# AlanLiangC/PDM-SSD

Measured on AMD Instinct MI355X. Metric: frames/sec (16384-pt clouds, bs=32), higher is better.
Workload: dtype f32; 1 GPU; configs[2]: full PDM-SSD forward (PointNet2MSG backbone + PDM neck + hybrid head: BEV heat-map head + point box head with decoded boxes), bs=32/GPU x 16384 pts, uniform KITTI-range clouds, fp32 inference, inputs resident in HBM, 4 distinct batches in rotation; launch=hipGraph, parallelism=dp1, global_batch=32

## Files before the change

### include/pdmssd_hip.h

```cpp
#ifndef PDMSSD_HIP_H
#define PDMSSD_HIP_H

#include <stddef.h>

#ifdef __cplusplus
extern "C" {
#endif

#define PDM_ABI_VERSION 1

#define PDM_E_BADARG (-1)
#define PDM_E_TOOLARGE (-2)

int pdm_abi_version(void);
const char *pdm_last_error(void);


int pdm_ball_query(void *stream, int b, int n, int m, float radius, int nsample,
                   const float *new_xyz, const float *xyz, int *idx);

int pdm_group_points(void *stream, int b, int c, int n, int npoints, int nsample,
                     const float *points, const int *idx, float *out);

int pdm_group_points_grad(void *stream, int b, int c, int n, int npoints, int nsample,
// ... 330 lines not shown
                        void *xmin, unsigned char *imax, unsigned char *imin);
int pdm_tg_dy_stats_parts(long long rows, int N);
int pdm_tg_gemm_nt_dy_bs(void *stream, long long R, int K, int N, const void *dZ, long long lddz, const void *Yp, long long ldyp,
                         const void *W, long long ldw, void *dX, long long lddx, void *dYout, long long lddy, const float *coef,
                         const float *grads, const void *Bx, long long ldbx, const float *bcoef, float *bstats);
size_t pdm_tg_wgrad_ws_bytes(long long R, int K, int N);
int pdm_tg_wgrad(void *stream, long long R, int K, int N, const void *dY, long long ldy, const void *X, long long ldx, float *dW,
                 int accumulate, void *workspace, size_t workspace_bytes, const float *x_bn_coef);
size_t pdm_tg_colsum_ws_floats(long long R, int N);
int pdm_tg_colsum(void *stream, long long R, int N, const void *Y, long long ld, float *out, float *scratch);
int pdm_tg_pack_weight(void *stream, int N, int K, const float *W, void *Wb, int ldb, void *Wt, int ldt);
int pdm_tg_pack_weight_pair(void *stream, int N, int K, const float *W, void *Wb, void *Wt, int rows_to, int cols_to);
int pdm_tg_pack_weight_many(void *stream, int njobs, const void *jobs, long long total_blocks);


int pdm_tune_fps_variant(int v);
int pdm_tune_fused_waves(int w);
int pdm_tune_fused_tiles(int t);
int pdm_tune_fused_groups(int n);
int pdm_tune_fused_wg_per_cu(int n);
int pdm_tune_fused_lds_cap(int bytes);
int pdm_tune_fused_reg(int on);
int pdm_tune_fused_gemm(int on);
int pdm_tune_fused_chain(int on);
int pdm_tune_fused_swz(int on);
int pdm_tune_bq_quad(int form);
int pdm_tune_bq_dense_ppc(int hundredths);
int pdm_tune_grid_split(int min_n);
int pdm_tune_bq_small_waves(int w);
int pdm_tune_bq_cpw(int centres);
int pdm_tune_bq_heavy(int candidates);
int pdm_tune_group_lds_floor(int bytes);
int pdm_tune_group_rows(int packed);
int pdm_tune_rows_chain_wg_per_cu(int n);
int pdm_tune_fp_head_tiles(int n);
int pdm_tune_rows_chain_dw_wg_per_cu(int n);
int pdm_tune_rows_chain_xcd(int on);
int pdm_tune_fp_chain_pad_lds(int bytes);

int pdm_copy_many(void *stream, int count, void *const *dst, const void *const *src, const size_t *bytes);
int pdm_copy_many_dyn(void *stream, int count, void *const *dst, const void *const *src, const size_t *bytes,
                      const int *const *dyn_count, const unsigned *dyn_unit);


int pdm_scatter_bev(void *stream, int B, int P, int C, int degree, const float *xyz,
                    const float *feat, const float *sh, const float *inv2s2, float ox, float oy,
// ... 37 lines not shown
```

### pdm_ssd_amd/_native.py

```python
import ctypes
import os

import torch

_HERE = os.path.dirname(os.path.abspath(__file__))
LIB_PATH = os.path.join(_HERE, "libpdmssd_hip.so")
ABI_VERSION = 1

_lib = None

_vp, _i, _f = ctypes.c_void_p, ctypes.c_int, ctypes.c_float

_SIGNATURES = {
    "pdm_ball_query": [_i, _i, _i, _f, _i, _vp, _vp, _vp],
    "pdm_ball_query_grid": [_i, _i, _i, _f, _i, _vp, _vp, _vp, _vp, ctypes.c_size_t],
    "pdm_grid_build": [_i, _i, _f, _vp, _vp, ctypes.c_size_t],
    "pdm_ball_query_grid_prebuilt": [_i, _i, _i, _f, _i, _vp, _vp, _vp, ctypes.c_size_t],
    "pdm_three_nn_grid_prebuilt": [_i, _i, _i, _vp, _vp, _vp, _vp, ctypes.c_size_t],
    "pdm_three_nn_grid": [_i, _i, _i, _vp, _vp, _vp, _vp, _vp, ctypes.c_size_t],
    "pdm_group_points": [_i, _i, _i, _i, _i, _vp, _vp, _vp],
    "pdm_group_points_grad": [_i, _i, _i, _i, _i, _vp, _vp, _vp],
    "pdm_group_points_grad_ws": [_i, _i, _i, _i, _i, _vp, _vp, _vp, _vp, ctypes.c_size_t],
    "pdm_gather_points": [_i, _i, _i, _i, _vp, _vp, _vp],
    "pdm_gather_points_grad": [_i, _i, _i, _i, _vp, _vp, _vp],
# ... 111 lines not shown
    "pdm_tg_colsum": [ctypes.c_longlong, _i, _vp, ctypes.c_longlong, _vp, _vp],
    "pdm_tg_pack_weight": [_i, _i, _vp, _vp, _i, _vp, _i],
    "pdm_tg_pack_weight_pair": [_i, _i, _vp, _vp, _vp, _i, _i],
    "pdm_tg_pack_weight_many": [_i, _vp, ctypes.c_longlong],
    "pdm_tune_fps_variant": None,
    "pdm_tune_fused_waves": None,
    "pdm_tune_fused_tiles": None,
    "pdm_tune_fused_groups": None,
    "pdm_tune_fused_wg_per_cu": None,
    "pdm_tune_fused_lds_cap": None,
    "pdm_tune_fused_reg": None,
    "pdm_tune_bq_quad": None,
    "pdm_tune_bq_heavy": None,
    "pdm_tune_bq_cpw": None,
    "pdm_tune_copy_variant": None,
    "pdm_tune_group_nt": None,
    "pdm_tune_group_lds_floor": None,
    "pdm_tune_copy_max_wg": None,
    "pdm_tune_bq_small_waves": None,
    "pdm_tune_bq_dense_ppc": None,
    "pdm_tune_grid_split": None,
    "pdm_tune_group_rows": None,
    "pdm_tune_fused_gemm": None,
    "pdm_tune_fused_chain": None,
    "pdm_tune_fused_pair": None,
    "pdm_tune_sa_pair": None,
    "pdm_tune_rows_x3_wg_per_cu": None,
    "pdm_tune_fp_chain_pad_lds": None,
    "pdm_tune_fp_chain_nt": None,
    "pdm_tune_fp_chain_mask": None,
    "pdm_tune_rows_chain_wg_per_cu": None,
    "pdm_tune_rows_chain_dw_wg_per_cu": None,
    "pdm_tune_fp_head_tiles": None,
    "pdm_tune_rows_chain_xcd": None,
    "pdm_tune_fused_swz": None,
    "pdm_scatter_bev": [_i, _i, _i, _i, _vp, _vp, _vp, _vp] + [_f] * 9 + [_i] * 7 + [_vp, _vp],
    "pdm_gather_bev": [_i, _i, _i, _i, _vp, _vp, _vp, _vp] + [_f] * 9 + [_i] * 6 + [_i, _f, _vp, _vp, _vp, ctypes.c_size_t],
    "pdm_bev_normalize_grad": [_i, _i, _i, _i, _i, _f, _vp, _vp, _vp, _vp, _vp],
    "pdm_bev_normalize": [_i, _i, _i, _i, _i, _i, _f, _vp, _vp],
    "pdm_scatter_bev_grad": [_i, _i, _i, _i, _vp, _vp, _vp, _vp] + [_f] * 9 + [_i] * 7 + [_vp] * 5,
    "pdm_scatter_bev_grad_normalized": [_i, _i, _i, _i, _vp, _vp, _vp, _vp] + [_f] * 9 + [_i] * 7 + [_vp, _vp, _f] + [_vp] * 4,
}
EXPORTS = ["pdm_abi_version", "pdm_last_error", "pdm_ball_query_grid_workspace_bytes",
           "pdm_three_nn_grid_workspace_bytes", "pdm_furthest_point_sampling_ws_bytes",
           "pdm_fps_max_coresident_workgroups",
           "pdm_gather_bev_workspace_bytes", "pdm_nms_workspace_bytes", "pdm_post_process_workspace_bytes", "pdm_augment_workspace_bytes", "pdm_kitti_eval_workspace_bytes", "pdm_kitti_data_fov_workspace_bytes",
           "pdm_kitti_data_boxes_workspace_bytes", "pdm_sa_pack_workspace_bytes",
           "pdm_sa_pack_rows", "pdm_rows_mlp_x3_stream_bytes", "pdm_point_head_loss_workspace_bytes", "pdm_heatmap_focal_loss_workspace_bytes", "pdm_three_interpolate_grad_ws_bytes",
           "pdm_group_points_grad_ws_bytes", "pdm_group_concat_cl_grad_ws_bytes", "pdm_bn_parts", "pdm_bn_pool_parts",
           "pdm_tg_stats_parts", "pdm_tg_dy_stats_parts", "pdm_tg_wgrad_ws_bytes", "pdm_tg_colsum_ws_floats"] + list(_SIGNATURES)


class NativeLibraryError(RuntimeError):
    pass


def lib():
    global _lib
    if _lib is None:
        if not os.path.exists(LIB_PATH):
            raise NativeLibraryError(
                f"{LIB_PATH} not found: build it with `make -C pdm_ssd_amd/csrc` "
                "(or `python -c 'import __graft_entry__ as g; g.build()'`). "
                "pdm_ssd_amd has no CPU or PyTorch fallback for its operators.")
        l = ctypes.CDLL(LIB_PATH)
        l.pdm_abi_version.restype = _i
        l.pdm_last_error.restype = ctypes.c_char_p
        l.pdm_ball_query_grid_workspace_bytes.restype = ctypes.c_size_t
        l.pdm_ball_query_grid_workspace_bytes.argtypes = [_i, _i]
        l.pdm_furthest_point_sampling_ws_bytes.restype = ctypes.c_size_t
        l.pdm_furthest_point_sampling_ws_bytes.argtypes = [_i, _i]
        l.pdm_fps_max_coresident_workgroups.restype = _i
        l.pdm_fps_max_coresident_workgroups.argtypes = []
        l.pdm_gather_bev_workspace_bytes.restype = ctypes.c_size_t
        l.pdm_gather_bev_workspace_bytes.argtypes = [_i] * 6
        l.pdm_three_nn_grid_workspace_bytes.restype = ctypes.c_size_t
        l.pdm_three_nn_grid_workspace_bytes.argtypes = [_i, _i]
        l.pdm_nms_workspace_bytes.restype = ctypes.c_size_t
        l.pdm_sa_pack_workspace_bytes.restype = ctypes.c_size_t
        l.pdm_sa_pack_workspace_bytes.argtypes = [_i, _i]
        l.pdm_group_concat_cl_grad_ws_bytes.restype = ctypes.c_size_t
        l.pdm_group_concat_cl_grad_ws_bytes.argtypes = [_i, _i, _i, _i]
        l.pdm_group_points_grad_ws_bytes.restype = ctypes.c_size_t
        l.pdm_group_points_grad_ws_bytes.argtypes = [_i, _i, _i, _i]
        l.pdm_three_interpolate_grad_ws_bytes.restype = ctypes.c_size_t
        l.pdm_three_interpolate_grad_ws_bytes.argtypes = [_i, _i, _i]
        l.pdm_point_head_loss_workspace_bytes.restype = ctypes.c_size_t
        l.pdm_point_head_loss_workspace_bytes.argtypes = [ctypes.c_longlong]
        l.pdm_heatmap_focal_loss_workspace_bytes.restype = ctypes.c_size_t
        l.pdm_heatmap_focal_loss_workspace_bytes.argtypes = [ctypes.c_longlong]
        l.pdm_rows_mlp_x3_stream_bytes.restype = ctypes.c_size_t
        l.pdm_rows_mlp_x3_stream_bytes.argtypes = [_i, _vp]
        l.pdm_sa_pack_rows.restype = ctypes.c_size_t
        l.pdm_sa_pack_rows.argtypes = [_i, _i, _i]
        l.pdm_nms_workspace_bytes.argtypes = [_i]
        l.pdm_post_process_workspace_bytes.restype = ctypes.c_size_t
# ... 102 lines not shown
```

### pdm_ssd_amd/csrc/fused_mlp.hip

```cpp
#include "common.h"

#include <mutex>
#include <set>

namespace pdm {

typedef float f4 __attribute__((ext_vector_type(4)));

constexpr int FM_MAXL = 4;

struct MlpDesc {
    int nlayers;
    int K[FM_MAXL + 1];
    int woff[FM_MAXL];
    int boff[FM_MAXL];
    int stage_in;
    int pool_floats;
    int relu_last;
    int lds_p, lds_q;
    int swz;
};

__device__ __forceinline__ int lds_col(int blk, int g, int pos, int swz) {
    const int q = 4 * blk + g;
// ... 976 lines not shown
            for (int t = 0; t < NT; ++t)
                if (orow[t]) sa_reg_store4(orow[t], 16 * mb + 4 * g, a.cout, v[t]);
        }
    }
}

int rows_gemm_launch(void *stream, int rows, int cin, const float *in_pm, int k0, int c1, const float *wpack,
                     const float *bias, int relu_last, float *out_pm, int out_stride, int cout);
int rows_chain_launch(void *stream, int rows, int cin, const float *in_pm, int nlayers, const int *dims, const float *wpack,
                      const float *bias, int relu_last, float *out_pm, int out_stride, int cout, int *launched);
int rows_chain_pair_launch(void *stream, int rows, int cin, const float *in_pm, int nlayers, const int *dims, const float *wpack_a,
                           const float *bias_a, const float *wpack_b, const float *bias_b, int relu_last, float *out_a, int out_stride_a,
                           int cout_a, float *out_b, int out_stride_b, int cout_b, int *launched);
static int g_fused_chain = 1;
static int g_fused_pair = 1;
int fp_chain_launch(void *stream, int b, int n, int m, int c_skip, const float *z_pm, int z_stride, const float *skip_pm,
                    const int *idx, const float *weight, const int *dims, const float *wpack, const float *bias, float *out_pm,
                    int out_stride, int cout, int *launched);
int fp_pre_gemm_launch(void *stream, int b, int n, int m, int c_skip, const float *z_pm, int z_stride,
                       const float *skip_pm, const int *idx, const float *weight, int k1, int c2,
                       const float *wpack, const float *bias, float *out_pm, int out_stride, int cout);
static int g_fused_swz = 1;
static int g_fused_gemm = 1;
static int g_fused_reg = 1;
static int g_fused_waves = 0;
static int g_fused_tiles = 0;
static int g_fused_groups = 0;
static int g_fused_lds_cap = 152 * 1024;
static int g_fused_wg_per_cu = 32;

static int fill_desc(const char *who, MlpDesc &d, int nlayers, const int *dims, int k0_real_max, int pool_floats,
                     long long ntiles, int *waves, int *tiles_per_wg, int *groups, bool two_tiles) {
    PDM_REQUIRE(nlayers >= 1 && nlayers <= FM_MAXL, PDM_E_BADARG, "%s: nlayers=%d not in [1,%d]", who, nlayers, FM_MAXL);
    PDM_REQUIRE(dims, PDM_E_BADARG, "%s: null dims", who);
    d.nlayers = nlayers;
    d.relu_last = 1;
    int wo = 0, bo = 0;
    for (int l = 0; l <= nlayers; ++l) {
        PDM_REQUIRE(dims[l] > 0 && dims[l] % 16 == 0, PDM_E_BADARG, "%s: padded width %d of level %d is not a positive multiple of 16", who, dims[l], l);
        d.K[l] = dims[l];
    }
    for (int l = 0; l < nlayers; ++l) {
        d.woff[l] = wo; d.boff[l] = bo;
        wo += d.K[l] * d.K[l + 1];
        bo += d.K[l + 1];
    }
// ... 20 lines not shown
    d.lds_q = roww(q);
    d.pool_floats = pool_floats;
    const int region_bytes = (NT * 16 * (d.lds_p + d.lds_q) + pool_floats) * 4;
    int G = NT == 2 ? 1 : (g_fused_groups > 0 ? g_fused_groups : W == 2 ? 2 : 1);
    while (G > 1 && (G * W > 8 || (long long)G * region_bytes > 64 * 1024 || (long long)G * NT * 4 > ntiles)) G >>= 1;
    *groups = G;
    return 0;
}

}

using namespace pdm;

extern "C" int pdm_tune_fused_waves(int w) { const int old = g_fused_waves; g_fused_waves = (w == 1 || w == 2 || w == 4 || w == 8) ? w : 0; return old; }

static void allow_lds(const void *fn, size_t bytes) {
    if (bytes > 64 * 1024) (void)grant_lds(fn, 160 * 1024);
}
extern "C" int pdm_tune_fused_lds_cap(int bytes) { const int old = g_fused_lds_cap; if (bytes >= 16 * 1024 && bytes <= 160 * 1024) g_fused_lds_cap = bytes; return old; }
extern "C" int pdm_tune_fused_swz(int on) { const int old = g_fused_swz; g_fused_swz = on != 0; return old; }
extern "C" int pdm_tune_fused_chain(int on) { const int old = g_fused_chain; g_fused_chain = on != 0; return old; }
extern "C" int pdm_tune_fused_pair(int on) { const int old = g_fused_pair; g_fused_pair = on != 0; return old; }
extern "C" int pdm_tune_fused_gemm(int on) { const int old = g_fused_gemm; g_fused_gemm = on != 0; return old; }
extern "C" int pdm_tune_fused_reg(int on) { const int old = g_fused_reg; g_fused_reg = on != 0; return old; }
extern "C" int pdm_tune_fused_wg_per_cu(int n) { const int old = g_fused_wg_per_cu; if (n > 0) g_fused_wg_per_cu = n; return old; }
extern "C" int pdm_tune_fused_groups(int n) { const int old = g_fused_groups; g_fused_groups = (n == 1 || n == 2 || n == 4 || n == 8) ? n : 0; return old; }
extern "C" int pdm_tune_fused_tiles(int t) { const int old = g_fused_tiles; g_fused_tiles = t; return old; }

#define FUSED_LAUNCH2(KERNEL, W, G, PRE, blocks, lds_bytes, ...)                                              \
    do {                                                                                                       \
        constexpr int MAXNB = (W <= 2) ? 2 : 4;      \
        if (NT == 2 && W >= 4 && G == 1) {                           \
            allow_lds(reinterpret_cast<const void *>(&KERNEL<(W >= 4 ? W : 4), 2, 2, 1, PRE>), lds_bytes);     \
            hipLaunchKernelGGL((KERNEL<(W >= 4 ? W : 4), 2, 2, 1, PRE>), dim3(blocks), dim3(64 * W * G),       \
                               lds_bytes, as_stream(stream), __VA_ARGS__);                                     \
        } else {                                                                                               \
            allow_lds(reinterpret_cast<const void *>(&KERNEL<W, 1, MAXNB, G, PRE>), lds_bytes);                \
            hipLaunchKernelGGL((KERNEL<W, 1, MAXNB, G, PRE>), dim3(blocks), dim3(64 * W * G), lds_bytes,       \
                               as_stream(stream), __VA_ARGS__);                                                \
        }                                                                                                      \
    } while (0)
#define FUSED_LAUNCH1(KERNEL, W, G, blocks, lds_bytes, ...)                                                   \
    do {                                                                                                       \
        if (pre_form) FUSED_LAUNCH2(KERNEL, W, G, true, blocks, lds_bytes, __VA_ARGS__);                       \
        else FUSED_LAUNCH2(KERNEL, W, G, false, blocks, lds_bytes, __VA_ARGS__);                               \
    } while (0)
// ... 199 lines not shown
    int rc = fill_desc("fp_mlp_fused", d, nlayers, dims, c_known + c_skip, 0, ntiles, &W, &NT, &G, mode == 1);
    if (rc) return rc;
    d.relu_last = relu_last ? 1 : 0;
    if (mode == 1)
        PDM_REQUIRE(z_stride % 4 == 0 && z_stride >= d.K[1] && (reinterpret_cast<uintptr_t>(z_pm) & 15) == 0, PDM_E_BADARG,
                    "fp_mlp_fused_pre: z rows need %d floats, stride %d, 16-byte aligned", d.K[1], z_stride);
    PDM_REQUIRE(cout > 0 && cout <= d.K[nlayers] && cout <= out_stride, PDM_E_BADARG, "fp_mlp_fused: cout=%d stride=%d", cout, out_stride);
    PDM_REQUIRE(out_stride % 4 == 0 && (reinterpret_cast<uintptr_t>(out_pm) & 15) == 0 &&
                    (reinterpret_cast<uintptr_t>(wpack) & 15) == 0 && (reinterpret_cast<uintptr_t>(bias) & 15) == 0 &&
                    (c_known % 4 != 0 || (reinterpret_cast<uintptr_t>(known_pm) & 15) == 0) &&
                    (c_skip % 4 != 0 || c_skip == 0 || (reinterpret_cast<uintptr_t>(skip_pm) & 15) == 0),
                PDM_E_BADARG, "fp_mlp_fused: buffers must be 16-byte aligned and out_stride a multiple of 4");
    FpArgs a{b, n, m, c_known, c_skip, known_pm, skip_pm, idx, weight, out_pm, out_stride, cout, mode == 1 ? z_pm : nullptr, z_stride};
    const bool pre_form = mode == 1;
    PDM_REQUIRE(!pre_form || (long long)m * z_stride < (1ll << 31), PDM_E_TOOLARGE, "fp_mlp_fused_pre: m * z_stride overflows 32-bit row offsets");
    if (g_fused_chain && pre_form && nlayers == 2 && z_stride >= d.K[1] &&
        (c_skip <= 4 || (c_skip % 4 == 0 && (reinterpret_cast<uintptr_t>(skip_pm) & 15) == 0))) {
        int launched = 0;
        const int crc = fp_chain_launch(stream, b, n, m, c_skip, z_pm, z_stride, skip_pm, idx, weight, dims, wpack, bias, out_pm,
                                        out_stride, cout, &launched);
        if (crc || launched) return crc;
    }
    if (g_fused_gemm && pre_form && nlayers == 2 && c_skip <= 4 && d.K[0] == 16 && d.K[1] >= 64 && d.K[2] >= 64 &&
        (long long)b * n >= 32768 && (long long)b * n < (1ll << 31) && z_stride >= d.K[1])
        return fp_pre_gemm_launch(stream, b, n, m, c_skip, z_pm, z_stride, skip_pm, idx, weight, d.K[1], d.K[2], wpack, bias,
                                  out_pm, out_stride, cout);
    const size_t lds_bytes = (size_t)G * (NT * 16 * (d.lds_p + d.lds_q)) * sizeof(float);
    PDM_REQUIRE(lds_bytes <= 160 * 1024, PDM_E_TOOLARGE, "fp_mlp_fused: needs %zu bytes of LDS", lds_bytes);
    const long long niter = ((ntiles + NT - 1) / NT + G - 1) / G;
    const long long cap = (long long)256 * g_fused_wg_per_cu;
    const int blocks = (int)(niter < cap ? niter : cap);
    FUSED_DISPATCH(fp_mlp_fused_kernel, W, G, blocks, lds_bytes, d, a, wpack, bias);
    return check_launch("fp_mlp_fused");
}

extern "C" int pdm_fp_mlp_fused(void *stream, int b, int n, int m, int c_known, int c_skip,
                                const float *known_pm, const float *skip_pm, const int *idx,
                                const float *weight, int nlayers, const int *dims, const float *wpack,
                                const float *bias, float *out_pm, int out_stride, int cout) {
    PDM_REQUIRE(c_known >= 1, PDM_E_BADARG, "fp_mlp_fused: c_known=%d", c_known);
    return fp_fused_launch(stream, 0, 1, b, n, m, c_known, c_skip, known_pm, nullptr, 0, skip_pm, idx, weight, nlayers,
                           dims, wpack, bias, out_pm, out_stride, cout);
}

extern "C" int pdm_fp_mlp_fused_pre(void *stream, int b, int n, int m, int c_skip, const float *z_pm,
                                    int z_stride, const float *skip_pm, const int *idx, const float *weight,
                                    int nlayers, const int *dims, const float *wpack, const float *bias,
                                    float *out_pm, int out_stride, int cout) {
    return fp_fused_launch(stream, 1, 1, b, n, m, 0, c_skip, nullptr, z_pm, z_stride, skip_pm, idx, weight, nlayers, dims,
                           wpack, bias, out_pm, out_stride, cout);
}

extern "C" int pdm_rows_mlp_fused(void *stream, int rows, int cin, const float *in_pm, int nlayers,
                                  const int *dims, const float *wpack, const float *bias, int relu_last,
                                  float *out_pm, int out_stride, int cout) {
    PDM_REQUIRE(rows >= 0 && cin >= 1, PDM_E_BADARG, "rows_mlp_fused: rows=%d cin=%d", rows, cin);
    if (g_fused_chain && dims && in_pm && wpack && bias && out_pm && cout > 0 && nlayers >= 1 && nlayers <= 3 && cout <= dims[nlayers] &&
        cout <= out_stride && out_stride % 4 == 0 &&
        ((reinterpret_cast<uintptr_t>(out_pm) | reinterpret_cast<uintptr_t>(wpack) | reinterpret_cast<uintptr_t>(bias) |
          reinterpret_cast<uintptr_t>(in_pm)) & 15) == 0) {
        int launched = 0;
        const int rc = rows_chain_launch(stream, rows, cin, in_pm, nlayers, dims, wpack, bias, relu_last, out_pm, out_stride, cout,
                                         &launched);
        if (rc || launched) return rc;
    }
    if (g_fused_gemm && nlayers == 1 && dims && dims[0] % 16 == 0 && dims[1] % 16 == 0 && dims[0] >= cin && dims[0] >= 32 &&
        dims[1] >= 64 && (long long)((rows + 127) / 128) * ((dims[1] + 127) / 128) >= 256 && in_pm && wpack && bias && out_pm && cout > 0 && cout <= dims[1] && cout <= out_stride &&
        out_stride % 4 == 0 && ((reinterpret_cast<uintptr_t>(out_pm) | reinterpret_cast<uintptr_t>(wpack) |
                                 reinterpret_cast<uintptr_t>(bias)) & 15) == 0)
        return rows_gemm_launch(stream, rows, cin, in_pm, dims[0], dims[1], wpack, bias, relu_last, out_pm, out_stride, cout);
    return fp_fused_launch(stream, 2, relu_last, 1, rows, 1, 0, cin, nullptr, nullptr, 0, in_pm, nullptr, nullptr, nlayers,
                           dims, wpack, bias, out_pm, out_stride, cout);
}

extern "C" int pdm_rows_mlp_fused_pair(void *stream, int rows, int cin, const float *in_pm, int nlayers, const int *dims,
                                       const float *wpack_a, const float *bias_a, const float *wpack_b, const float *bias_b,
                                       int relu_last, float *out_a, int out_stride_a, int cout_a, float *out_b, int out_stride_b,
                                       int cout_b) {
    PDM_REQUIRE(rows >= 0 && cin >= 1, PDM_E_BADARG, "rows_mlp_fused_pair: rows=%d cin=%d", rows, cin);
    if (g_fused_chain && g_fused_pair && dims && in_pm && wpack_a && bias_a && wpack_b && bias_b && out_a && out_b && out_a != out_b &&
        nlayers == 3 && cout_a > 0 && cout_b > 0 && cout_a <= dims[nlayers] && cout_b <= dims[nlayers] && cout_a <= out_stride_a &&
        cout_b <= out_stride_b && out_stride_a % 4 == 0 && out_stride_b % 4 == 0 &&
        ((reinterpret_cast<uintptr_t>(out_a) | reinterpret_cast<uintptr_t>(out_b) | reinterpret_cast<uintptr_t>(wpack_a) |
          reinterpret_cast<uintptr_t>(wpack_b) | reinterpret_cast<uintptr_t>(bias_a) | reinterpret_cast<uintptr_t>(bias_b) |
          reinterpret_cast<uintptr_t>(in_pm)) & 15) == 0) {
        int launched = 0;
        const int rc = rows_chain_pair_launch(stream, rows, cin, in_pm, nlayers, dims, wpack_a, bias_a, wpack_b, bias_b, relu_last, out_a,
                                              out_stride_a, cout_a, out_b, out_stride_b, cout_b, &launched);
        if (rc || launched) return rc;
    }
// ... 4 lines not shown
```

### pdm_ssd_amd/csrc/rows_gemm.hip

```cpp
#include "common.h"

namespace pdm {

typedef float gf4 __attribute__((ext_vector_type(4)));

constexpr int RG_ROWS = 128;
constexpr int RG_BLKS = 8;
constexpr int RG_HS = 24;

struct RowsGemmArgs {
    int rows, cin, in_stride;
    int nkb, nmb;
    int cout, out_stride;
    const float *in;
    const float *wpack;
    const float *bias;
    float *out;
    float floor;
    int n, m, z_stride, c_skip;
    const float *z;
    const float *skip;
    const int *idx;
    const float *weight;
    const float *w1;
    const float *b1;
};

template <bool FP_PRE>
__global__ __launch_bounds__(512) void rows_gemm_kernel(RowsGemmArgs a) {
    __shared__ __attribute__((aligned(16))) float s_w[2][RG_BLKS * 64 * 4];
    __shared__ __attribute__((aligned(16))) float s_h[2][RG_ROWS * RG_HS];
    const int tid = threadIdx.x, lane = tid & 63;
    const int wave = __builtin_amdgcn_readfirstlane(tid >> 6);
    const int pos = lane & 15, g = lane >> 4;
    const int wp = wave >> 2, wc = wave & 3;
    int tile = blockIdx.x;
    if constexpr (FP_PRE) {
        const int tpc = a.n / RG_ROWS, nb = a.rows / a.n;
        if (gridDim.y == 1 && tpc * RG_ROWS == a.n && (nb & 7) == 0) {
            const int xcd = tile & 7, slot = tile >> 3;
            tile = ((slot / tpc) * 8 + xcd) * tpc + slot % tpc;
        }
    }
    const long long r0 = (long long)tile * RG_ROWS;
    const int mb0 = blockIdx.y * RG_BLKS;

    const int hrow = tid >> 2, part = tid & 3;
    const bool w_live = mb0 + wave < a.nmb;
    const gf4 *wsrc = reinterpret_cast<const gf4 *>(a.wpack) + ((size_t)(mb0 + wave) * a.nkb) * 64 + lane;
    const bool h_live = r0 + hrow < a.rows;
    const float *hsrc = a.in + (size_t)(r0 + hrow) * a.in_stride + 4 * part;
    const bool vec = (a.in_stride & 3) == 0 && (reinterpret_cast<uintptr_t>(a.in) & 15) == 0;

    auto load_w = [&](int kb) {
        gf4 v = {0.f, 0.f, 0.f, 0.f};
        if (w_live) v = wsrc[(size_t)kb * 64];
        return v;
    };
    const float *zb = nullptr;
    int o0 = 0, o1 = 0, o2 = 0;
    float iw0 = 0.f, iw1 = 0.f, iw2 = 0.f, sk[4] = {0.f, 0.f, 0.f, 0.f};
    if constexpr (FP_PRE) {
        if (h_live) {
            const long long row = r0 + hrow;
            const int b = (int)(row / a.n);
            zb = a.z + (size_t)b * a.m * a.z_stride + 4 * part;
            o0 = a.idx[row * 3] * a.z_stride; o1 = a.idx[row * 3 + 1] * a.z_stride; o2 = a.idx[row * 3 + 2] * a.z_stride;
            iw0 = a.weight[row * 3]; iw1 = a.weight[row * 3 + 1]; iw2 = a.weight[row * 3 + 2];
            for (int s_ = 0; s_ < a.c_skip; ++s_) sk[s_] = a.skip[row * a.c_skip + s_];
        }
    }
    struct Raw { gf4 za, zc, zd; };
    auto load_raw = [&](int kb) {
        Raw r;
        r.za = r.zc = r.zd = gf4{0.f, 0.f, 0.f, 0.f};
        if (h_live) {
            r.za = *reinterpret_cast<const gf4 *>(zb + o0 + 16 * kb);
            r.zc = *reinterpret_cast<const gf4 *>(zb + o1 + 16 * kb);
            r.zd = *reinterpret_cast<const gf4 *>(zb + o2 + 16 * kb);
        }
        return r;
    };
    auto finish = [&](const Raw &r, int kb) {
        gf4 v = {0.f, 0.f, 0.f, 0.f};
        if (!h_live) return v;
        const int c = 16 * kb + 4 * part;
        const gf4 bb = *reinterpret_cast<const gf4 *>(a.b1 + c);
        float h[4] = {bb.x, bb.y, bb.z, bb.w};
        const float zz[3][4] = {{r.za.x, r.za.y, r.za.z, r.za.w}, {r.zc.x, r.zc.y, r.zc.z, r.zc.w}, {r.zd.x, r.zd.y, r.zd.z, r.zd.w}};
#pragma unroll
        for (int j = 0; j < 4; ++j) {
            h[j] += __fmaf_rn(iw2, zz[2][j], __fmaf_rn(iw1, zz[1][j], __fmul_rn(iw0, zz[0][j])));
            const float *wr = a.w1 + ((size_t)(c >> 4) * 64 + ((c & 15) + j)) * 4;
            for (int s_ = 0; s_ < a.c_skip; ++s_) h[j] = fmaf(wr[s_], sk[s_], h[j]);
            h[j] = fmaxf(h[j], 0.0f);
        }
        return gf4{h[0], h[1], h[2], h[3]};
    };
    auto load_h = [&](int kb) {
        gf4 v = {0.f, 0.f, 0.f, 0.f};
        if (!h_live) return v;
        const int c = 16 * kb + 4 * part;
        if (vec && c + 4 <= a.cin) return *reinterpret_cast<const gf4 *>(hsrc + 16 * kb);
        const float *p = hsrc + 16 * kb;
        if (c < a.cin) v.x = p[0];
        if (c + 1 < a.cin) v.y = p[1];
        if (c + 2 < a.cin) v.z = p[2];
        if (c + 3 < a.cin) v.w = p[3];
        return v;
    };
    auto stage = [&](int buf, gf4 w, gf4 h) {
        reinterpret_cast<gf4 *>(s_w[buf])[tid] = w;
        *reinterpret_cast<gf4 *>(&s_h[buf][hrow * RG_HS + 4 * part]) = h;
    };

    gf4 acc[2][4];
#pragma unroll
    for (int i = 0; i < 2; ++i) {
        gf4 bi = {0.f, 0.f, 0.f, 0.f};
        if (mb0 + 2 * wc + i < a.nmb) bi = *reinterpret_cast<const gf4 *>(a.bias + 16 * (mb0 + 2 * wc + i) + 4 * g);
#pragma unroll
        for (int t = 0; t < 4; ++t) acc[i][t] = bi;
    }

    gf4 gw = load_w(0), gh = {0.f, 0.f, 0.f, 0.f};
    Raw gr;
    if constexpr (FP_PRE) { gr = load_raw(0); gh = finish(gr, 0); } else gh = load_h(0);
    stage(0, gw, gh);
    __syncthreads();
    if (a.nkb > 1) {
        gw = load_w(1);
        if constexpr (FP_PRE) gr = load_raw(1); else gh = load_h(1);
    }
    for (int kb = 0; kb < a.nkb; ++kb) {
        const int cur = kb & 1;
        gf4 fa[2], fb[4];
#pragma unroll
        for (int i = 0; i < 2; ++i) fa[i] = reinterpret_cast<const gf4 *>(s_w[cur])[(2 * wc + i) * 64 + lane];
#pragma unroll
        for (int t = 0; t < 4; ++t) fb[t] = *reinterpret_cast<const gf4 *>(&s_h[cur][((4 * wp + t) * 16 + pos) * RG_HS + 4 * g]);
        if (kb + 1 < a.nkb) {
            if constexpr (FP_PRE) gh = finish(gr, kb + 1);
            stage(cur ^ 1, gw, gh);
        }
        if (kb + 2 < a.nkb) {
            gw = load_w(kb + 2);
            if constexpr (FP_PRE) gr = load_raw(kb + 2); else gh = load_h(kb + 2);
        }
#define PDM_RG_MFMA(C)                                                                                         \
    _Pragma("unroll") for (int i = 0; i < 2; ++i) _Pragma("unroll") for (int t = 0; t < 4; ++t)                 \
        acc[i][t] = __builtin_amdgcn_mfma_f32_16x16x4f32(fa[i].C, fb[t].C, acc[i][t], 0, 0, 0);
        PDM_RG_MFMA(x) PDM_RG_MFMA(y) PDM_RG_MFMA(z) PDM_RG_MFMA(w)
#undef PDM_RG_MFMA
        __syncthreads();
    }

#pragma unroll
    for (int t = 0; t < 4; ++t) {
        const long long row = r0 + (4 * wp + t) * 16 + pos;
        if (row >= a.rows) continue;
        float *orow = a.out + (size_t)row * a.out_stride;
#pragma unroll
        for (int i = 0; i < 2; ++i) {
            const int c0 = 16 * (mb0 + 2 * wc + i) + 4 * g;
            gf4 v = acc[i][t];
            v.x = __builtin_amdgcn_fmed3f(v.x, a.floor, __builtin_inff()); v.y = __builtin_amdgcn_fmed3f(v.y, a.floor, __builtin_inff());
            v.z = __builtin_amdgcn_fmed3f(v.z, a.floor, __builtin_inff()); v.w = __builtin_amdgcn_fmed3f(v.w, a.floor, __builtin_inff());
            if (c0 + 4 <= a.cout) {
                *reinterpret_cast<gf4 *>(orow + c0) = v;
            } else {
                if (c0 < a.cout) orow[c0] = v.x;
                if (c0 + 1 < a.cout) orow[c0 + 1] = v.y;
                if (c0 + 2 < a.cout) orow[c0 + 2] = v.z;
            }
        }
    }
}

int rows_gemm_launch(void *stream, int rows, int cin, const float *in_pm, int k0, int c1, const float *wpack,
                     const float *bias, int relu_last, float *out_pm, int out_stride, int cout) {
    RowsGemmArgs a;
    a.rows = rows; a.cin = cin; a.in_stride = cin;
    a.nkb = k0 >> 4; a.nmb = c1 >> 4;
    a.cout = cout; a.out_stride = out_stride;
    a.in = in_pm; a.wpack = wpack; a.bias = bias; a.out = out_pm;
    a.floor = relu_last ? 0.0f : -__builtin_inff();
    a.n = a.m = a.z_stride = a.c_skip = 0;
    a.z = a.skip = a.weight = a.w1 = a.b1 = nullptr; a.idx = nullptr;
    const dim3 grid((unsigned)((rows + RG_ROWS - 1) / RG_ROWS), (unsigned)((a.nmb + RG_BLKS - 1) / RG_BLKS));
    hipLaunchKernelGGL(rows_gemm_kernel<false>, grid, dim3(512), 0, as_stream(stream), a);
    return check_launch("rows_mlp_fused(gemm)");
}

int fp_pre_gemm_launch(void *stream, int b, int n, int m, int c_skip, const float *z_pm, int z_stride,
                       const float *skip_pm, const int *idx, const float *weight, int k1, int c2,
                       const float *wpack, const float *bias, float *out_pm, int out_stride, int cout) {
    RowsGemmArgs a;
    a.rows = b * n; a.cin = k1; a.in_stride = 0;
    a.nkb = k1 >> 4; a.nmb = c2 >> 4;
    a.cout = cout; a.out_stride = out_stride;
    a.in = nullptr; a.wpack = wpack + 16 * k1; a.bias = bias + k1; a.out = out_pm;
    a.floor = 0.0f;
    a.n = n; a.m = m; a.z_stride = z_stride; a.c_skip = c_skip;
    a.z = z_pm; a.skip = skip_pm; a.idx = idx; a.weight = weight; a.w1 = wpack; a.b1 = bias;
    const dim3 grid((unsigned)((a.rows + RG_ROWS - 1) / RG_ROWS), (unsigned)((a.nmb + RG_BLKS - 1) / RG_BLKS));
    hipLaunchKernelGGL(rows_gemm_kernel<true>, grid, dim3(512), 0, as_stream(stream), a);
    return check_launch("fp_mlp_fused_pre(gemm)");
}

}
```

Baseline: 7257 frames/s.

## Make rows GEMM kernel persistent with cross-tile software pipelining

```diff
diff --git a/include/pdmssd_hip.h b/include/pdmssd_hip.h
--- a/include/pdmssd_hip.h
+++ b/include/pdmssd_hip.h
@@ -376,6 +376,9 @@
 int pdm_tune_fused_lds_cap(int bytes);
 int pdm_tune_fused_reg(int on);
 int pdm_tune_fused_gemm(int on);
+int pdm_tune_rows_gemm_grid(int n);
+int pdm_rows_gemm_launches(void);
+int pdm_tune_rows_gemm_min_tiles(int n);
 int pdm_tune_fused_chain(int on);
 int pdm_tune_fused_swz(int on);
 int pdm_tune_bq_quad(int form);
diff --git a/pdm_ssd_amd/_native.py b/pdm_ssd_amd/_native.py
--- a/pdm_ssd_amd/_native.py
+++ b/pdm_ssd_amd/_native.py
@@ -157,6 +157,8 @@
     "pdm_tune_grid_split": None,
     "pdm_tune_group_rows": None,
     "pdm_tune_fused_gemm": None,
+    "pdm_tune_rows_gemm_grid": None,
+    "pdm_tune_rows_gemm_min_tiles": None,
     "pdm_tune_fused_chain": None,
     "pdm_tune_fused_pair": None,
     "pdm_tune_sa_pair": None,
@@ -178,7 +180,7 @@
 }
 EXPORTS = ["pdm_abi_version", "pdm_last_error", "pdm_ball_query_grid_workspace_bytes",
            "pdm_three_nn_grid_workspace_bytes", "pdm_furthest_point_sampling_ws_bytes",
-           "pdm_fps_max_coresident_workgroups",
+           "pdm_fps_max_coresident_workgroups", "pdm_rows_gemm_launches",
            "pdm_gather_bev_workspace_bytes", "pdm_nms_workspace_bytes", "pdm_post_process_workspace_bytes", "pdm_augment_workspace_bytes", "pdm_kitti_eval_workspace_bytes", "pdm_kitti_data_fov_workspace_bytes",
            "pdm_kitti_data_boxes_workspace_bytes", "pdm_sa_pack_workspace_bytes",
            "pdm_sa_pack_rows", "pdm_rows_mlp_x3_stream_bytes", "pdm_point_head_loss_workspace_bytes", "pdm_heatmap_focal_loss_workspace_bytes", "pdm_three_interpolate_grad_ws_bytes",
@@ -207,6 +209,8 @@
         l.pdm_furthest_point_sampling_ws_bytes.argtypes = [_i, _i]
         l.pdm_fps_max_coresident_workgroups.restype = _i
         l.pdm_fps_max_coresident_workgroups.argtypes = []
+        l.pdm_rows_gemm_launches.restype = _i
+        l.pdm_rows_gemm_launches.argtypes = []
         l.pdm_gather_bev_workspace_bytes.restype = ctypes.c_size_t
         l.pdm_gather_bev_workspace_bytes.argtypes = [_i] * 6
         l.pdm_three_nn_grid_workspace_bytes.restype = ctypes.c_size_t
diff --git a/pdm_ssd_amd/csrc/fused_mlp.hip b/pdm_ssd_amd/csrc/fused_mlp.hip
--- a/pdm_ssd_amd/csrc/fused_mlp.hip
+++ b/pdm_ssd_amd/csrc/fused_mlp.hip
@@ -1022,6 +1022,7 @@
                        const float *wpack, const float *bias, float *out_pm, int out_stride, int cout);
 static int g_fused_swz = 1;
 static int g_fused_gemm = 1;
+static int g_gemm_min_tiles = 256;
 static int g_fused_reg = 1;
 static int g_fused_waves = 0;
 static int g_fused_tiles = 0;
@@ -1088,6 +1089,7 @@
 extern "C" int pdm_tune_fused_chain(int on) { const int old = g_fused_chain; g_fused_chain = on != 0; return old; }
 extern "C" int pdm_tune_fused_pair(int on) { const int old = g_fused_pair; g_fused_pair = on != 0; return old; }
 extern "C" int pdm_tune_fused_gemm(int on) { const int old = g_fused_gemm; g_fused_gemm = on != 0; return old; }
+extern "C" int pdm_tune_rows_gemm_min_tiles(int n) { const int old = g_gemm_min_tiles; g_gemm_min_tiles = n > 0 ? n : 256; return old; }
 extern "C" int pdm_tune_fused_reg(int on) { const int old = g_fused_reg; g_fused_reg = on != 0; return old; }
 extern "C" int pdm_tune_fused_wg_per_cu(int n) { const int old = g_fused_wg_per_cu; if (n > 0) g_fused_wg_per_cu = n; return old; }
 extern "C" int pdm_tune_fused_groups(int n) { const int old = g_fused_groups; g_fused_groups = (n == 1 || n == 2 || n == 4 || n == 8) ? n : 0; return old; }
@@ -1333,7 +1335,7 @@
         if (crc || launched) return crc;
     }
     if (g_fused_gemm && pre_form && nlayers == 2 && c_skip <= 4 && d.K[0] == 16 && d.K[1] >= 64 && d.K[2] >= 64 &&
-        (long long)b * n >= 32768 && (long long)b * n < (1ll << 31) && z_stride >= d.K[1])
+        (long long)b * n >= 128ll * g_gemm_min_tiles && (long long)b * n < (1ll << 31) && z_stride >= d.K[1])
         return fp_pre_gemm_launch(stream, b, n, m, c_skip, z_pm, z_stride, skip_pm, idx, weight, d.K[1], d.K[2], wpack, bias,
                                   out_pm, out_stride, cout);
     const size_t lds_bytes = (size_t)G * (NT * 16 * (d.lds_p + d.lds_q)) * sizeof(float);
@@ -1376,7 +1378,7 @@
         if (rc || launched) return rc;
     }
     if (g_fused_gemm && nlayers == 1 && dims && dims[0] % 16 == 0 && dims[1] % 16 == 0 && dims[0] >= cin && dims[0] >= 32 &&
-        dims[1] >= 64 && (long long)((rows + 127) / 128) * ((dims[1] + 127) / 128) >= 256 && in_pm && wpack && bias && out_pm && cout > 0 && cout <= dims[1] && cout <= out_stride &&
+        dims[1] >= 64 && (long long)((rows + 127) / 128) * ((dims[1] + 127) / 128) >= g_gemm_min_tiles && in_pm && wpack && bias && out_pm && cout > 0 && cout <= dims[1] && cout <= out_stride &&
         out_stride % 4 == 0 && ((reinterpret_cast<uintptr_t>(out_pm) | reinterpret_cast<uintptr_t>(wpack) |
                                  reinterpret_cast<uintptr_t>(bias)) & 15) == 0)
         return rows_gemm_launch(stream, rows, cin, in_pm, dims[0], dims[1], wpack, bias, relu_last, out_pm, out_stride, cout);
diff --git a/pdm_ssd_amd/csrc/rows_gemm.hip b/pdm_ssd_amd/csrc/rows_gemm.hip
--- a/pdm_ssd_amd/csrc/rows_gemm.hip
+++ b/pdm_ssd_amd/csrc/rows_gemm.hip
@@ -3,6 +3,26 @@
 namespace pdm {
 
 typedef float gf4 __attribute__((ext_vector_type(4)));
+typedef int gi3 __attribute__((ext_vector_type(3)));
+typedef int gi3u __attribute__((ext_vector_type(3), aligned(4)));
+
+#ifndef RG_DIAG
+#define RG_DIAG 0
+#endif
+#if RG_DIAG
+#define RG_STAMP(i)                                                                                  \
+    do {                                                                                             \
+        __builtin_amdgcn_sched_barrier(0);                                                           \
+        unsigned long long t_;                                                                       \
+        asm volatile("s_memtime %0\n\ts_waitcnt lgkmcnt(0)" : "=s"(t_)::"memory");                   \
+        __builtin_amdgcn_sched_barrier(0);                                                           \
+        d_sum[i] += t_ - d_last;                                                                     \
+        d_last = t_;                                                                                 \
+    } while (0)
+#else
+#define RG_STAMP(i) do { } while (0)
+#endif
+enum { RG_PH_COLD, RG_PH_STAGE, RG_PH_REQUEST, RG_PH_MFMA, RG_PH_BARRIER, RG_PH_EPILOGUE, RG_PH_N };
 
 constexpr int RG_ROWS = 128;
 constexpr int RG_BLKS = 8;
@@ -24,82 +44,101 @@
     const float *weight;
     const float *w1;
     const float *b1;
+    int ncol, tiles, xcd;
 };
 
 template <bool FP_PRE>
-__global__ __launch_bounds__(512) void rows_gemm_kernel(RowsGemmArgs a) {
+__global__ __launch_bounds__(512, 4) void rows_gemm_kernel(RowsGemmArgs a) {
     __shared__ __attribute__((aligned(16))) float s_w[2][RG_BLKS * 64 * 4];
     __shared__ __attribute__((aligned(16))) float s_h[2][RG_ROWS * RG_HS];
+    __shared__ __attribute__((aligned(16))) float s_bias[2][16 * RG_BLKS];
     const int tid = threadIdx.x, lane = tid & 63;
     const int wave = __builtin_amdgcn_readfirstlane(tid >> 6);
     const int pos = lane & 15, g = lane >> 4;
     const int wp = wave >> 2, wc = wave & 3;
-    int tile = blockIdx.x;
-    if constexpr (FP_PRE) {
-        const int tpc = a.n / RG_ROWS, nb = a.rows / a.n;
-        if (gridDim.y == 1 && tpc * RG_ROWS == a.n && (nb & 7) == 0) {
-            const int xcd = tile & 7, slot = tile >> 3;
-            tile = ((slot / tpc) * 8 + xcd) * tpc + slot % tpc;
-        }
+    const int G = gridDim.x, wg = blockIdx.x;
+    int first, count, stride;
+    if (a.xcd) {
+        const int gx = G >> 3, slots = a.tiles >> 3;
+        first = wg >> 3; stride = gx; count = (slots - first + gx - 1) / gx;
+    } else {
+        first = (int)((long long)wg * a.tiles / G);
+        count = (int)((long long)(wg + 1) * a.tiles / G) - first; stride = 1;
     }
-    const long long r0 = (long long)tile * RG_ROWS;
-    const int mb0 = blockIdx.y * RG_BLKS;
+    const int tpc = FP_PRE && a.xcd ? a.n / RG_ROWS : 1;
+    auto tile_of = [&](int i, long long &r0, int &mb0) {
+        const int p = first + i * stride;
+        if (a.xcd) { r0 = (long long)(((p / tpc) * 8 + (wg & 7)) * tpc + p % tpc) * RG_ROWS; mb0 = 0; }
+        else { r0 = (long long)(p / a.ncol) * RG_ROWS; mb0 = (p % a.ncol) * RG_BLKS; }
+    };
 
     const int hrow = tid >> 2, part = tid & 3;
-    const bool w_live = mb0 + wave < a.nmb;
-    const gf4 *wsrc = reinterpret_cast<const gf4 *>(a.wpack) + ((size_t)(mb0 + wave) * a.nkb) * 64 + lane;
-    const bool h_live = r0 + hrow < a.rows;
-    const float *hsrc = a.in + (size_t)(r0 + hrow) * a.in_stride + 4 * part;
     const bool vec = (a.in_stride & 3) == 0 && (reinterpret_cast<uintptr_t>(a.in) & 15) == 0;
-
-    auto load_w = [&](int kb) {
-        gf4 v = {0.f, 0.f, 0.f, 0.f};
-        if (w_live) v = wsrc[(size_t)kb * 64];
-        return v;
-    };
+    const gf4 *wsrc = nullptr;
+    const float *hsrc = nullptr;
     const float *zb = nullptr;
     int o0 = 0, o1 = 0, o2 = 0;
+    gi3 ni = {0, 0, 0};
+    float gb = 0.f;
     float iw0 = 0.f, iw1 = 0.f, iw2 = 0.f, sk[4] = {0.f, 0.f, 0.f, 0.f};
-    if constexpr (FP_PRE) {
-        if (h_live) {
-            const long long row = r0 + hrow;
-            const int b = (int)(row / a.n);
-            zb = a.z + (size_t)b * a.m * a.z_stride + 4 * part;
-            o0 = a.idx[row * 3] * a.z_stride; o1 = a.idx[row * 3 + 1] * a.z_stride; o2 = a.idx[row * 3 + 2] * a.z_stride;
+
+    auto load_idx = [&](int i) {
+        long long r0; int mb0;
+        tile_of(i, r0, mb0);
+        const long long row = r0 + hrow < a.rows ? r0 + hrow : a.rows - 1;
+        ni = *reinterpret_cast<const gi3u *>(a.idx + row * 3);
+    };
+    auto enter = [&](int i) {
+        long long r0; int mb0;
+        tile_of(i, r0, mb0);
+        const int mb = mb0 + wave < a.nmb ? mb0 + wave : a.nmb - 1;
+        wsrc = reinterpret_cast<const gf4 *>(a.wpack) + ((size_t)mb * a.nkb) * 64 + lane;
+        const long long row = r0 + hrow < a.rows ? r0 + hrow : a.rows - 1;
+        const int bc = 16 * mb0 + (tid & (16 * RG_BLKS - 1));
+        if constexpr (FP_PRE) {
+            o0 = ni.x * a.z_stride; o1 = ni.y * a.z_stride; o2 = ni.z * a.z_stride;
+            zb = a.z + (size_t)((int)row / a.n) * a.m * a.z_stride + 4 * part;
+            gb = a.bias[bc < 16 * a.nmb ? bc : 16 * a.nmb - 1];
             iw0 = a.weight[row * 3]; iw1 = a.weight[row * 3 + 1]; iw2 = a.weight[row * 3 + 2];
-            for (int s_ = 0; s_ < a.c_skip; ++s_) sk[s_] = a.skip[row * a.c_skip + s_];
+#pragma unroll
+            for (int s_ = 0; s_ < 4; ++s_)
+                if (s_ < a.c_skip) sk[s_] = a.skip[row * a.c_skip + s_];
+        } else {
+            gb = a.bias[bc < 16 * a.nmb ? bc : 16 * a.nmb - 1];
+            hsrc = a.in + (size_t)row * a.in_stride + 4 * part;
         }
-    }
+    };
+    auto load_w = [&](int kb) {
+        return wsrc[(size_t)kb * 64];
+    };
     struct Raw { gf4 za, zc, zd; };
     auto load_raw = [&](int kb) {
         Raw r;
-        r.za = r.zc = r.zd = gf4{0.f, 0.f, 0.f, 0.f};
-        if (h_live) {
-            r.za = *reinterpret_cast<const gf4 *>(zb + o0 + 16 * kb);
-            r.zc = *reinterpret_cast<const gf4 *>(zb + o1 + 16 * kb);
-            r.zd = *reinterpret_cast<const gf4 *>(zb + o2 + 16 * kb);
-        }
+        r.za = *reinterpret_cast<const gf4 *>(zb + o0 + 16 * kb);
+        r.zc = *reinterpret_cast<const gf4 *>(zb + o1 + 16 * kb);
+        r.zd = *reinterpret_cast<const gf4 *>(zb + o2 + 16 * kb);
         return r;
     };
     auto finish = [&](const Raw &r, int kb) {
-        gf4 v = {0.f, 0.f, 0.f, 0.f};
-        if (!h_live) return v;
         const int c = 16 * kb + 4 * part;
         const gf4 bb = *reinterpret_cast<const gf4 *>(a.b1 + c);
         float h[4] = {bb.x, bb.y, bb.z, bb.w};
+        const gf4 *wr = reinterpret_cast<const gf4 *>(a.w1) + (size_t)(c >> 4) * 64 + (c & 15);
+        const gf4 w1r[4] = {wr[0], wr[1], wr[2], wr[3]};
         const float zz[3][4] = {{r.za.x, r.za.y, r.za.z, r.za.w}, {r.zc.x, r.zc.y, r.zc.z, r.zc.w}, {r.zd.x, r.zd.y, r.zd.z, r.zd.w}};
 #pragma unroll
         for (int j = 0; j < 4; ++j) {
             h[j] += __fmaf_rn(iw2, zz[2][j], __fmaf_rn(iw1, zz[1][j], __fmul_rn(iw0, zz[0][j])));
-            const float *wr = a.w1 + ((size_t)(c >> 4) * 64 + ((c & 15) + j)) * 4;
-            for (int s_ = 0; s_ < a.c_skip; ++s_) h[j] = fmaf(wr[s_], sk[s_], h[j]);
+            const float w1j[4] = {w1r[j].x, w1r[j].y, w1r[j].z, w1r[j].w};
+#pragma unroll
+            for (int s_ = 0; s_ < 4; ++s_)
+                if (s_ < a.c_skip) h[j] = fmaf(w1j[s_], sk[s_], h[j]);
             h[j] = fmaxf(h[j], 0.0f);
         }
         return gf4{h[0], h[1], h[2], h[3]};
     };
     auto load_h = [&](int kb) {
         gf4 v = {0.f, 0.f, 0.f, 0.f};
-        if (!h_live) return v;
         const int c = 16 * kb + 4 * part;
         if (vec && c + 4 <= a.cin) return *reinterpret_cast<const gf4 *>(hsrc + 16 * kb);
         const float *p = hsrc + 16 * kb;
@@ -114,67 +153,145 @@
         *reinterpret_cast<gf4 *>(&s_h[buf][hrow * RG_HS + 4 * part]) = h;
     };
 
+    gf4 gw = {0.f, 0.f, 0.f, 0.f}, gh = {0.f, 0.f, 0.f, 0.f};
+    Raw gr;
+    gr.za = gr.zc = gr.zd = gf4{0.f, 0.f, 0.f, 0.f};
+    int l_tile = 0, l_kb = 0, f_kb = 0;
+    auto request = [&]() {
+        if (l_kb == 0) enter(l_tile < count ? l_tile : count - 1);
+        gw = load_w(l_kb);
+        if constexpr (FP_PRE) gr = load_raw(l_kb); else gh = load_h(l_kb);
+        if (++l_kb == a.nkb) {
+            l_kb = 0; ++l_tile;
+            if constexpr (FP_PRE) load_idx(l_tile < count ? l_tile : count - 1);
+        }
+    };
+    auto write_stage = [&](int buf) {
+        if constexpr (FP_PRE) gh = finish(gr, f_kb);
+        stage(buf, gw, gh);
+        if (f_kb == 0 && tid < 16 * RG_BLKS) s_bias[buf][tid] = gb;
+        if (++f_kb == a.nkb) f_kb = 0;
+    };
+
+    long long r0;
+    int mb0;
+    tile_of(0, r0, mb0);
+    if (count <= 0) return;
+#if RG_DIAG
+    unsigned long long d_sum[RG_PH_N] = {0, 0, 0, 0, 0, 0}, d_last = __builtin_amdgcn_s_memtime();
+    const unsigned long long d_first = d_last;
+#endif
+    const int steps = count * a.nkb;
+    if constexpr (FP_PRE) load_idx(0);
+    request();
+    write_stage(0);
+    request();
+    __syncthreads();
+    RG_STAMP(RG_PH_COLD);
     gf4 acc[2][4];
 #pragma unroll
-    for (int i = 0; i < 2; ++i) {
-        gf4 bi = {0.f, 0.f, 0.f, 0.f};
-        if (mb0 + 2 * wc + i < a.nmb) bi = *reinterpret_cast<const gf4 *>(a.bias + 16 * (mb0 + 2 * wc + i) + 4 * g);
-#pragma unroll
-        for (int t = 0; t < 4; ++t) acc[i][t] = bi;
-    }
-
-    gf4 gw = load_w(0), gh = {0.f, 0.f, 0.f, 0.f};
-    Raw gr;
-    if constexpr (FP_PRE) { gr = load_raw(0); gh = finish(gr, 0); } else gh = load_h(0);
-    stage(0, gw, gh);
-    __syncthreads();
-    if (a.nkb > 1) {
-        gw = load_w(1);
-        if constexpr (FP_PRE) gr = load_raw(1); else gh = load_h(1);
-    }
-    for (int kb = 0; kb < a.nkb; ++kb) {
-        const int cur = kb & 1;
+    for (int i = 0; i < 2; ++i)
+#pragma unroll
+        for (int t = 0; t < 4; ++t) acc[i][t] = *reinterpret_cast<const gf4 *>(&s_bias[0][16 * (2 * wc + i) + 4 * g]);
+    int cur = 0, c_kb = 0, c_tile = 0;
+    for (int s = 0; s < steps; ++s, cur ^= 1) {
+        write_stage(cur ^ 1);
+        RG_STAMP(RG_PH_STAGE);
+        request();
+        RG_STAMP(RG_PH_REQUEST);
         gf4 fa[2], fb[4];
 #pragma unroll
         for (int i = 0; i < 2; ++i) fa[i] = reinterpret_cast<const gf4 *>(s_w[cur])[(2 * wc + i) * 64 + lane];
 #pragma unroll
         for (int t = 0; t < 4; ++t) fb[t] = *reinterpret_cast<const gf4 *>(&s_h[cur][((4 * wp + t) * 16 + pos) * RG_HS + 4 * g]);
-        if (kb + 1 < a.nkb) {
-            if constexpr (FP_PRE) gh = finish(gr, kb + 1);
-            stage(cur ^ 1, gw, gh);
-        }
-        if (kb + 2 < a.nkb) {
-            gw = load_w(kb + 2);
-            if constexpr (FP_PRE) gr = load_raw(kb + 2); else gh = load_h(kb + 2);
-        }
 #define PDM_RG_MFMA(C)                                                                                         \
     _Pragma("unroll") for (int i = 0; i < 2; ++i) _Pragma("unroll") for (int t = 0; t < 4; ++t)                 \
         acc[i][t] = __builtin_amdgcn_mfma_f32_16x16x4f32(fa[i].C, fb[t].C, acc[i][t], 0, 0, 0);
         PDM_RG_MFMA(x) PDM_RG_MFMA(y) PDM_RG_MFMA(z) PDM_RG_MFMA(w)
 #undef PDM_RG_MFMA
+        RG_STAMP(RG_PH_MFMA);
         __syncthreads();
-    }
-
-#pragma unroll
-    for (int t = 0; t < 4; ++t) {
-        const long long row = r0 + (4 * wp + t) * 16 + pos;
-        if (row >= a.rows) continue;
-        float *orow = a.out + (size_t)row * a.out_stride;
-#pragma unroll
-        for (int i = 0; i < 2; ++i) {
-            const int c0 = 16 * (mb0 + 2 * wc + i) + 4 * g;
-            gf4 v = acc[i][t];
-            v.x = __builtin_amdgcn_fmed3f(v.x, a.floor, __builtin_inff()); v.y = __builtin_amdgcn_fmed3f(v.y, a.floor, __builtin_inff());
-            v.z = __builtin_amdgcn_fmed3f(v.z, a.floor, __builtin_inff()); v.w = __builtin_amdgcn_fmed3f(v.w, a.floor, __builtin_inff());
-            if (c0 + 4 <= a.cout) {
-                *reinterpret_cast<gf4 *>(orow + c0) = v;
-            } else {
-                if (c0 < a.cout) orow[c0] = v.x;
-                if (c0 + 1 < a.cout) orow[c0 + 1] = v.y;
-                if (c0 + 2 < a.cout) orow[c0 + 2] = v.z;
+        RG_STAMP(RG_PH_BARRIER);
+        if (++c_kb < a.nkb) continue;
+
+        gf4 nbias[2];
+#pragma unroll
+        for (int i = 0; i < 2; ++i) nbias[i] = *reinterpret_cast<const gf4 *>(&s_bias[cur ^ 1][16 * (2 * wc + i) + 4 * g]);
+#pragma unroll
+        for (int t = 0; t < 4; ++t) {
+            const long long row = r0 + (4 * wp + t) * 16 + pos;
+            gf4 v[2];
+#pragma unroll
+            for (int i = 0; i < 2; ++i) {
+                v[i] = acc[i][t];
+                v[i].x = __builtin_amdgcn_fmed3f(v[i].x, a.floor, __builtin_inff()); v[i].y = __builtin_amdgcn_fmed3f(v[i].y, a.floor, __builtin_inff());
+                v[i].z = __builtin_amdgcn_fmed3f(v[i].z, a.floor, __builtin_inff()); v[i].w = __builtin_amdgcn_fmed3f(v[i].w, a.floor, __builtin_inff());
+                acc[i][t] = nbias[i];
+            }
+            if (row >= a.rows) continue;
+            float *orow = a.out + (size_t)row * a.out_stride;
+#pragma unroll
+            for (int i = 0; i < 2; ++i) {
+                const int c0 = 16 * (mb0 + 2 * wc + i) + 4 * g;
+                if (c0 + 4 <= a.cout) {
+                    *reinterpret_cast<gf4 *>(orow + c0) = v[i];
+                } else {
+                    if (c0 < a.cout) orow[c0] = v[i].x;
+                    if (c0 + 1 < a.cout) orow[c0 + 1] = v[i].y;
+                    if (c0 + 2 < a.cout) orow[c0 + 2] = v[i].z;
+                }
             }
         }
+        c_kb = 0;
+        if (++c_tile < count) tile_of(c_tile, r0, mb0);
+        RG_STAMP(RG_PH_EPILOGUE);
     }
+#if RG_DIAG
+    if (tid == 0) {
+        unsigned long long *d_out = reinterpret_cast<unsigned long long *>(a.out + (size_t)a.rows * a.out_stride) + (size_t)wg * 8;
+        for (int i = 0; i < RG_PH_N; ++i) d_out[i] = d_sum[i];
+        d_out[6] = d_first;
+        d_out[7] = d_last;
+    }
+#endif
+}
+
+static int g_rg_grid = 0;
+static int g_rg_launches = 0;
+
+template <bool FP_PRE>
+static int rg_resident_workgroups() {
+    static int cached[64] = {0};
+    int dev = 0;
+    if (hipGetDevice(&dev) != hipSuccess || dev < 0 || dev >= 64) return 0;
+    if (cached[dev] > 0) return cached[dev];
+    int cus = 0, per_cu = 0;
+    if (hipDeviceGetAttribute(&cus, hipDeviceAttributeMultiprocessorCount, dev) != hipSuccess) return 0;
+    if (hipOccupancyMaxActiveBlocksPerMultiprocessor(&per_cu, rows_gemm_kernel<FP_PRE>, 512, 0) != hipSuccess) return 0;
+    cached[dev] = cus * per_cu;
+    return cached[dev];
+}
+
+constexpr int RG_WALKS_PER_SLOT = 4;
+
+template <bool FP_PRE>
+static int rg_launch(void *stream, RowsGemmArgs &a, const char *what) {
+    a.ncol = (a.nmb + RG_BLKS - 1) / RG_BLKS;
+    const long long tiles = (long long)((a.rows + RG_ROWS - 1) / RG_ROWS) * a.ncol;
+    PDM_REQUIRE(tiles * a.nkb < (1ll << 31), PDM_E_TOOLARGE, "%s: %lld tiles of %d k-blocks overflow the 32-bit step count", what, tiles, a.nkb);
+    a.tiles = (int)tiles;
+    const long long resident = (long long)RG_WALKS_PER_SLOT * rg_resident_workgroups<FP_PRE>();
+    PDM_REQUIRE(resident > 0, (int)hipErrorUnknown, "%s: the runtime gives no resident-workgroup count", what);
+    long long grid = tiles < resident ? tiles : resident;
+    if (g_rg_grid > 0 && grid > g_rg_grid) grid = g_rg_grid;
+    a.xcd = 0;
+    if (FP_PRE && a.ncol == 1 && a.n % RG_ROWS == 0 && ((a.rows / a.n) & 7) == 0 && grid >= 8) {
+        a.xcd = 1;
+        grid &= ~7ll;
+    }
+    hipLaunchKernelGGL(rows_gemm_kernel<FP_PRE>, dim3((unsigned)grid), dim3(512), 0, as_stream(stream), a);
+    g_rg_launches = (g_rg_launches + 1) & 0x7fffffff;
+    return check_launch(what);
 }
 
 int rows_gemm_launch(void *stream, int rows, int cin, const float *in_pm, int k0, int c1, const float *wpack,
@@ -187,9 +304,7 @@
     a.floor = relu_last ? 0.0f : -__builtin_inff();
     a.n = a.m = a.z_stride = a.c_skip = 0;
     a.z = a.skip = a.weight = a.w1 = a.b1 = nullptr; a.idx = nullptr;
-    const dim3 grid((unsigned)((rows + RG_ROWS - 1) / RG_ROWS), (unsigned)((a.nmb + RG_BLKS - 1) / RG_BLKS));
-    hipLaunchKernelGGL(rows_gemm_kernel<false>, grid, dim3(512), 0, as_stream(stream), a);
-    return check_launch("rows_mlp_fused(gemm)");
+    return rg_launch<false>(stream, a, "rows_mlp_fused(gemm)");
 }
 
 int fp_pre_gemm_launch(void *stream, int b, int n, int m, int c_skip, const float *z_pm, int z_stride,
@@ -203,9 +318,10 @@
     a.floor = 0.0f;
     a.n = n; a.m = m; a.z_stride = z_stride; a.c_skip = c_skip;
     a.z = z_pm; a.skip = skip_pm; a.idx = idx; a.weight = weight; a.w1 = wpack; a.b1 = bias;
-    const dim3 grid((unsigned)((a.rows + RG_ROWS - 1) / RG_ROWS), (unsigned)((a.nmb + RG_BLKS - 1) / RG_BLKS));
-    hipLaunchKernelGGL(rows_gemm_kernel<true>, grid, dim3(512), 0, as_stream(stream), a);
-    return check_launch("fp_mlp_fused_pre(gemm)");
-}
-
-}
+    return rg_launch<true>(stream, a, "fp_mlp_fused_pre(gemm)");
+}
+
+}
+
+extern "C" int pdm_rows_gemm_launches(void) { return pdm::g_rg_launches; }
+extern "C" int pdm_tune_rows_gemm_grid(int n) { const int old = pdm::g_rg_grid; pdm::g_rg_grid = n > 0 ? n : 0; return old; }
```

Result: no change. 7239 frames/s (-0.3%).
